# nianticlabs/simplerecon

Measured on AMD Instinct MI355X. Metric: depth frames/sec (640x480, 7 src views, 64 planes), higher is better.
Workload: dtype f32

## Files before the change

include/simplerecon_hip.h:

```cpp
#ifndef SIMPLERECON_HIP_H_
#define SIMPLERECON_HIP_H_

#include <stddef.h>
#include <stdint.h>

#ifdef __cplusplus
extern "C" {
#endif

#define SR_OK 0
#define SR_ERR_INVALID_ARGUMENT 1
#define SR_ERR_UNSUPPORTED 2
#define SR_ERR_WORKSPACE_TOO_SMALL 3
#define SR_ERR_HIP_BASE 1000

enum {
  SR_OPT_MLP_SPLIT = 0, SR_OPT_WINO_SPLIT, SR_OPT_WINO_XCD, SR_OPT_WINO_NT, SR_OPT_WINO_KSPLIT, SR_OPT_CONV_WINO,
  SR_OPT_CONV_TILE, SR_OPT_CONV_KSPLIT, SR_OPT_PW_NT, SR_OPT_PW_KS, SR_OPT_PT_CFG, SR_OPT_PT_KS, SR_OPT_DOT_LDS,
  SR_OPT_DOT_LDS_G, SR_OPT_DOT_LDS_CULL, SR_OPT_DOT_LDS_CAP, SR_OPT_UPSAMPLE_QUAD, SR_OPT_POOL_STREAM,
  SR_OPT_MLP_TILE,
  SR_OPT_COUNT
};
int sr_option_count(void);
const char* sr_option_name(int id);
int sr_option_id(const char* name);
int sr_option_get(int id, int* value);
int sr_option_set(int id, int value, int* previous );
int sr_option_default(int id, int* value);

int sr_abi_version(void);

const char* sr_target_arch(void);


size_t sr_volume_workspace_bytes(int B, int K, int C, int h, int w);

int sr_volume_prepare(const float* src, const float* K_src, const float* T_src_cur,
                      const float* T_cur_src, int B, int K, int C, int h, int w, void* workspace,
                      size_t workspace_bytes, void* stream);

int sr_dot_volume_sweep(const float* cur, const float* invK_cur, const float* planes, int64_t ps_b,
                        int64_t ps_d, int64_t ps_y, int64_t ps_x, int B, int K, int C, int h, int w,
                        int D, float* out_cv, int64_t cv_sb, int64_t cv_sd, int64_t cv_sp,
                        float* out_lowest, uint8_t* out_mask, void* workspace,
                        size_t workspace_bytes, void* stream);

int sr_conv3x3_wino_io_nhwc_fwd(const void* in, int64_t in_batch_stride, int in_pix_stride, const float* packed_u,
                                const float* bias, const void* residual, int64_t res_batch_stride, int res_pix_stride,
                                void* out, int64_t out_batch_stride, int out_pix_stride, int B, int H, int W, int Cin,
                                int Cout, float leaky_slope, int io_dtype, void* stream);
int sr_pw_conv_io_nhwc_fwd(const void* in, int64_t in_batch_stride, int in_pix_stride, const float* packed_w,
                           const float* bias, const void* residual, int64_t res_batch_stride, int res_pix_stride, void* out,
                           int64_t out_batch_stride, int out_pix_stride, int B, int HW, int Cin, int Cout, float act_code,
                           int io_dtype, void* stream);

size_t sr_pw_conv_tiled_workspace_bytes(int M, int Cin, int Cout);
int sr_pw_conv_tiled_plan(int M, int Cin, int Cout, int can_split, int* cfg, int* ks);
int sr_pw_conv_tiled_nhwc_fwd(const float* in, int in_pix_stride, const float* packed_w, const float* bias,
                              const float* gate, const float* residual, int res_pix_stride, float* out,
                              int out_pix_stride, int M, int HW, int Cin, int Cout, float act_code, void* workspace,
                              size_t workspace_bytes, void* stream);
int sr_pw_conv_supported(int Cin, int Cout);
int sr_pw_conv_plan(int B, int HW, int Cin, int Cout, int* nt, int* ks);
int sr_pw_conv_nhwc_fwd(const float* in, int64_t in_batch_stride, int in_pix_stride, const float* packed_w,
                        const float* bias, const float* gate, const float* residual, int64_t res_batch_stride,
                        int res_pix_stride, float* out, int64_t out_batch_stride, int out_pix_stride, int B, int HW,
                        int Cin, int Cout, float act_code, void* stream);

int sr_backproject_fwd(const float* depth, const float* invK, float* out_points, int B, int h, int w, void* stream);
int sr_project3d_fwd(const float* points, const float* K, const float* T, float* out, int B, int N, float eps,
                     void* stream);
int sr_backproject_bwd(const float* grad_points, const float* invK, float* grad_depth, int B, int h, int w, void* stream);
int sr_project3d_bwd(const float* grad_out, const float* points, const float* K, const float* T, float* grad_points, int B,
                     int N, float eps, void* stream);
int sr_pose_distance_fwd(const float* T, float* out, int n, void* stream);
int sr_camera_rays_fwd(const float* points, const float* T, float* out, int B, int N, int in_camera_frame, void* stream);

int sr_selftest_rcp(const float* x, float* out_fast, float* out_div, int n, void* stream);

int sr_dot_volume_fwd(const float* cur, const float* src, const float* K_src,
                      const float* T_src_cur, const float* invK_cur, const float* planes,
                      int64_t ps_b, int64_t ps_d, int64_t ps_y, int64_t ps_x, int B, int K, int C,
                      int h, int w, int D, float* out_cv, int64_t cv_sb, int64_t cv_sd,
                      int64_t cv_sp, float* out_lowest, uint8_t* out_mask, void* workspace,
                      size_t workspace_bytes, void* stream);

int sr_warp_features_fwd(const float* src, const float* K_src, const float* T_src_cur,
                         const float* invK_cur, const float* planes, int64_t ps_b, int64_t ps_d,
                         int64_t ps_y, int64_t ps_x, int B, int K, int C, int h, int w, int Dp,
                         float* out_world, float* out_depths, float* out_warped, float* out_mask,
                         float* out_pix, void* workspace, size_t workspace_bytes, void* stream);

size_t sr_mlp_volume_workspace_bytes(int B, int K, int C, int h, int w, int hidden);

int sr_mlp_pack_weights(const float* W1, const float* b1, const float* W2, const float* b2,
                        const float* W3, const float* b3, int hidden, int B, int K, int C, int h, int w,
                        void* workspace, size_t workspace_bytes, void* stream);

int sr_mlp_volume_sweep(const float* cur, const float* invK_cur, const float* planes, int64_t ps_b,
                        int64_t ps_d, int64_t ps_y, int64_t ps_x, float leaky_slope, int B, int K,
                        int C, int h, int w, int D, float* out_cv, int64_t cv_sb, int64_t cv_sd,
                        int64_t cv_sp, float* out_lowest, uint8_t* out_mask, void* workspace,
                        size_t workspace_bytes, void* stream);

int sr_mlp_volume_tile_shape(int h, int w, int* th, int* tw);

int sr_mlp_volume_fwd(const float* cur, const float* src, const float* K_src, const float* T_src_cur,
                      const float* T_cur_src, const float* invK_cur, const float* planes, int64_t ps_b,
                      int64_t ps_d, int64_t ps_y, int64_t ps_x, const float* W1, const float* b1,
                      const float* W2, const float* b2, const float* W3, const float* b3, int hidden,
                      float leaky_slope, int B, int K, int C, int h, int w, int D, float* out_cv,
                      int64_t cv_sb, int64_t cv_sd, int64_t cv_sp, float* out_lowest, uint8_t* out_mask,
                      int reserve_cus, void* workspace, size_t workspace_bytes, void* stream);


size_t sr_conv_packed_weight_floats(int Cout, int Cin, int ksize);

int sr_conv_pack_weights(const float* weight, int Cout, int Cin, int ksize, float* packed, void* stream);

int sr_conv2d_nhwc_fwd(const float* in, int64_t in_batch_stride, int in_pix_stride,
                       const float* packed_weight, const float* bias, const float* residual,
                       int64_t res_batch_stride, int res_pix_stride, float* out,
                       int64_t out_batch_stride, int out_pix_stride, int B, int H, int W, int Cin,
                       int Cout, int ksize, int stride, float leaky_slope, void* stream);

int sr_conv2d_replicate_nhwc_fwd(const float* in, int64_t in_batch_stride, int in_pix_stride,
                                 const float* packed_weight, const float* bias, const float* residual,
                                 int64_t res_batch_stride, int res_pix_stride, float* out,
                                 int64_t out_batch_stride, int out_pix_stride, int B, int H, int W, int Cin,
                                 int Cout, int ksize, int stride, float leaky_slope, void* stream);

#define SR_ACT_NONE (-1.0f)
#define SR_ACT_SILU (-2.0f)
int sr_conv2d_padded_nhwc_fwd(const float* in, int64_t in_batch_stride, int in_pix_stride,
                              const float* packed_weight, const float* bias, const float* residual,
                              int64_t res_batch_stride, int res_pix_stride, float* out,
                              int64_t out_batch_stride, int out_pix_stride, int B, int H, int W, int Cin,
                              int Cout, int ksize, int stride, int pad_top, int pad_left, int pad_bottom,
                              int pad_right, float leaky_slope, void* stream);

size_t sr_conv_splitk_workspace_bytes(int B, int H, int W, int Cin, int Cout, int ksize, int stride);
int sr_conv2d_splitk_nhwc_fwd(const float* in, int64_t in_batch_stride, int in_pix_stride,
                              const float* packed_weight, const float* bias, const float* residual,
                              int64_t res_batch_stride, int res_pix_stride, float* out,
                              int64_t out_batch_stride, int out_pix_stride, int B, int H, int W, int Cin,
                              int Cout, int ksize, int stride, float leaky_slope, void* workspace,
                              size_t workspace_bytes, void* stream);

size_t sr_wino_packed_weight_floats(int Cout, int Cin);
int sr_wino_pack_weights(const float* weight, int Cout, int Cin, float* packed, void* stream);
int sr_conv_prefers_wino(int B, int H, int W, int Cin, int Cout, int ksize, int stride);
int sr_conv3x3_wino_nhwc_fwd(const float* in, int64_t in_batch_stride, int in_pix_stride,
                             const float* packed_u, const float* bias, const float* residual,
                             int64_t res_batch_stride, int res_pix_stride, float* out,
                             int64_t out_batch_stride, int out_pix_stride, int B, int H, int W, int Cin,
                             int Cout, float leaky_slope, void* stream);

size_t sr_wino4_packed_weight_floats(int Cout, int Cin);
// ... 392 lines not shown
```

simplerecon_amd/_lib.py:

```python
import contextlib
import ctypes as C
import os

import torch

_HERE = os.path.dirname(os.path.abspath(__file__))
LIB_PATH = os.environ.get("SR_HIP_LIBRARY") or os.path.join(_HERE, "libsimplerecon_hip.so")
ABI_VERSION = 3

_lib = None

_p = C.c_void_p
_i = C.c_int
_i64 = C.c_int64
_f = C.c_float
_sz = C.c_size_t

SIGNATURES = {
    "sr_abi_version": (_i, []),
    "sr_option_count": (_i, []),
    "sr_option_name": (C.c_char_p, [_i]),
    "sr_option_id": (_i, [C.c_char_p]),
    "sr_option_get": (_i, [_i, C.POINTER(C.c_int)]),
    "sr_option_set": (_i, [_i, _i, C.POINTER(C.c_int)]),
    "sr_option_default": (_i, [_i, C.POINTER(C.c_int)]),
    "sr_target_arch": (C.c_char_p, []),
    "sr_volume_workspace_bytes": (_sz, [_i, _i, _i, _i, _i]),
    "sr_volume_prepare": (_i, [_p, _p, _p, _p, _i, _i, _i, _i, _i, _p, _sz, _p]),
    "sr_dot_volume_sweep": (_i, [_p, _p, _p, _i64, _i64, _i64, _i64, _i, _i, _i, _i, _i, _i,
                                 _p, _i64, _i64, _i64, _p, _p, _p, _sz, _p]),
    "sr_dot_volume_fwd": (_i, [_p, _p, _p, _p, _p, _p, _i64, _i64, _i64, _i64, _i, _i, _i, _i, _i, _i,
                               _p, _i64, _i64, _i64, _p, _p, _p, _sz, _p]),
    "sr_rgb_stem3x3s2_fwd": (_i, [_p, _i64, _i64, _i64, _i64, _p, _p, _p, _i64, _i, _i, _i, _i, _i, _i, _i, _i, _i, _f, _p]),
    "sr_se_gate2_fwd": (_i, [_p, _i, _i, _p, _p, _p, _p, _p, _p, _i, _i, _i, _p]),
    "sr_conv3x3_wino_io_nhwc_fwd": (_i, [_p, _i64, _i, _p, _p, _p, _i64, _i, _p, _i64, _i, _i, _i, _i, _i, _i, _f, _i, _p]),
    "sr_pw_conv_io_nhwc_fwd": (_i, [_p, _i64, _i, _p, _p, _p, _i64, _i, _p, _i64, _i, _i, _i, _i, _i, _f, _i, _p]),
    "sr_conv16_packed_weight_bytes": (_sz, [_i, _i, _i]),
    "sr_conv16_pack_weights": (_i, [_p, _i, _i, _i, _i, _p, _p]),
    "sr_conv16_supported": (_i, [_i, _i, _i, _i, _i, _i, _i]),
    "sr_conv16_prefers": (_i, [_i, _i, _i, _i, _i, _i, _i]),
    "sr_conv16_nhwc_fwd": (_i, [_p, _i64, _i, _p, _p, _p, _i64, _i, _p, _i64, _i, _i, _i, _i, _i, _i, _i, _i, _f, _i, _i, _p]),
    "sr_conv16_wgrad_supported": (_i, [_i, _i, _i, _i, _i, _i, _i]),
    "sr_conv16_wgrad_prefers": (_i, [_i, _i, _i, _i, _i, _i, _i]),
    "sr_conv16_wgrad_workspace_bytes": (_sz, [_i, _i, _i, _i, _i, _i, _i]),
    "sr_conv16_wgrad_nhwc": (_i, [_p, _i64, _i, _p, _i64, _i, _p, _i, _i, _i, _i, _i, _i, _i, _i, _p, _sz, _p]),
    "sr_act_bwd_bias16_workspace_bytes": (_sz, [_i64, _i]),
    "sr_act_bwd_bias16_nhwc": (_i, [_p, _i, _p, _p, _p, _i64, _i, _f, _i, _p, _sz, _p]),
    "sr_pw_conv_tiled_workspace_bytes": (_sz, [_i, _i, _i]),
    "sr_pw_conv_tiled_plan": (_i, [_i, _i, _i, _i, _p, _p]),
    "sr_pw_conv_tiled_nhwc_fwd": (_i, [_p, _i, _p, _p, _p, _p, _i, _p, _i, _i, _i, _i, _i, _f, _p, _sz, _p]),
    "sr_pw_conv_supported": (_i, [_i, _i]),
    "sr_pw_conv_plan": (_i, [_i, _i, _i, _i, _p, _p]),
    "sr_pw_conv_nhwc_fwd": (_i, [_p, _i64, _i, _p, _p, _p, _p, _i64, _i, _p, _i64, _i, _i, _i, _i, _i, _f, _p]),
    "sr_backproject_fwd": (_i, [_p, _p, _p, _i, _i, _i, _p]),
    "sr_project3d_fwd": (_i, [_p, _p, _p, _p, _i, _i, _f, _p]),
    "sr_backproject_bwd": (_i, [_p, _p, _p, _i, _i, _i, _p]),
    "sr_project3d_bwd": (_i, [_p, _p, _p, _p, _p, _i, _i, _f, _p]),
    "sr_pose_distance_fwd": (_i, [_p, _p, _i, _p]),
    "sr_camera_rays_fwd": (_i, [_p, _p, _p, _i, _i, _i, _p]),
    "sr_selftest_rcp": (_i, [_p, _p, _p, _i, _p]),
    "sr_warp_features_fwd": (_i, [_p, _p, _p, _p, _p, _i64, _i64, _i64, _i64, _i, _i, _i, _i, _i, _i,
                                  _p, _p, _p, _p, _p, _p, _sz, _p]),
    "sr_mlp_volume_workspace_bytes": (_sz, [_i, _i, _i, _i, _i, _i]),
    "sr_mlp_pack_weights": (_i, [_p, _p, _p, _p, _p, _p, _i, _i, _i, _i, _i, _i, _p, _sz, _p]),
    "sr_mlp_volume_sweep": (_i, [_p, _p, _p, _i64, _i64, _i64, _i64, _f, _i, _i, _i, _i, _i, _i,
                                 _p, _i64, _i64, _i64, _p, _p, _p, _sz, _p]),
    "sr_mlp_volume_tile_shape": (_i, [_i, _i, C.POINTER(C.c_int), C.POINTER(C.c_int)]),
    "sr_mlp_volume_fwd": (_i, [_p, _p, _p, _p, _p, _p, _p, _i64, _i64, _i64, _i64, _p, _p, _p, _p, _p, _p, _i,
                               _f, _i, _i, _i, _i, _i, _i, _p, _i64, _i64, _i64, _p, _p, _i, _p, _sz, _p]),
    "sr_conv_packed_weight_floats": (_sz, [_i, _i, _i]),
    "sr_conv_pack_weights": (_i, [_p, _i, _i, _i, _p, _p]),
    "sr_conv2d_nhwc_fwd": (_i, [_p, _i64, _i, _p, _p, _p, _i64, _i, _p, _i64, _i, _i, _i, _i, _i, _i, _i, _i, _f, _p]),
    "sr_conv2d_replicate_nhwc_fwd": (_i, [_p, _i64, _i, _p, _p, _p, _i64, _i, _p, _i64, _i, _i, _i, _i, _i, _i, _i, _i,
                                          _f, _p]),
    "sr_conv2d_padded_nhwc_fwd": (_i, [_p, _i64, _i, _p, _p, _p, _i64, _i, _p, _i64, _i, _i, _i, _i, _i, _i, _i, _i,
                                       _i, _i, _i, _i, _f, _p]),
    "sr_dwconv3x3_pool_bands": (_i, [_i]),
    "sr_dwconv3x3_nhwc_fwd": (_i, [_p, _i64, _i, _p, _p, _p, _i64, _i, _p, _i, _i, _i, _i, _i, _i, _i, _i, _i, _f,
                                   _p]),
    "sr_add_nhwc_fwd": (_i, [_p, _i64, _i, _p, _i64, _i, _p, _i64, _i, _i, _i, _i, _i, _p]),
    "sr_se_scale_nhwc_fwd": (_i, [_p, _i, _p, _p, _p, _p, _p, _p, _i64, _i, _p, _i64, _i, _p, _i, _i, _i, _i, _i,
                                  _p]),
    "sr_se_gate_fwd": (_i, [_p, _i, _i, _p, _p, _p, _p, _p, _i, _i, _i, _p]),
    "sr_scale_channels_nhwc_fwd": (_i, [_p, _i64, _i, _p, _p, _i64, _i, _i, _i, _i, _i, _p]),
    "sr_dot_volume_bwd_scratch_bytes": (_sz, [_i, _i, _i, _i, _i]),
    "sr_dot_volume_bwd": (_i, [_p, _i64, _i64, _i64, _p, _p, _p, _i64, _i64, _i64, _i64, _i, _i, _i, _i, _i, _i, _p, _p,
                               _p, _sz, _p, _sz, _p]),
    "sr_mlp_volume_bwd_scratch_bytes": (_sz, [_i, _i, _i, _i, _i, _i]),
    "sr_mlp_volume_bwd": (_i, [_p, _i64, _i64, _i64, _p, _p, _p, _i64, _i64, _i64, _i64, _p, _p, _p, _p, _p, _f, _i, _i,
                               _i, _i, _i, _i, _i, _p, _p, _p, _p, _p, _p, _p, _p, _p, _sz, _p, _sz, _p]),
    "sr_conv_wgrad_workspace_bytes": (_sz, [_i, _i, _i, _i, _i, _i, _i]),
    "sr_conv_wgrad_nhwc": (_i, [_p, _i64, _i, _p, _i64, _i, _p, _i, _i, _i, _i, _i, _i, _i, _p, _sz, _p]),
    "sr_bias_grad_nhwc": (_i, [_p, _i64, _i, _p, _i, _i, _i, _i, _p]),
    "sr_act_bwd": (_i, [_p, _p, _p, _i64, _f, _p]),
    "sr_act_bwd_bias_workspace_bytes": (_sz, [_i64, _i]),
    "sr_act_bwd_bias_nhwc": (_i, [_p, _p, _p, _p, _i64, _i, _f, _p, _sz, _p]),
    "sr_zero_stuff2x_nhwc": (_i, [_p, _i64, _i, _p, _i, _i, _i, _i, _i, _i, _p]),
    "sr_upsample2x_bwd_nhwc": (_i, [_p, _i64, _i, _p, _i64, _i, _i, _i, _i, _i, _p]),
    "sr_conv_flip_transpose_weights": (_i, [_p, _i, _i, _i, _p, _p]),
    "sr_mul_fwd": (_i, [_p, _p, _p, _i64, _p]),
    "sr_norm_workspace_bytes": (_sz, [_i, _i, _i, _i]),
    "sr_norm_stats_nhwc": (_i, [_p, _i64, _i, _i, _i, _i, _i, _p, _p, _p, _sz, _p]),
    "sr_norm_act_fwd_nhwc": (_i, [_p, _i64, _i, _p, _p, _f, _p, _p, _f, _i, _p, _i64, _i, _i, _i, _i, _p]),
    "sr_norm_act_bwd_nhwc": (_i, [_p, _i64, _i, _p, _i64, _i, _p, _p, _f, _p, _p, _f, _i, _i, _p, _i64, _i, _p, _p,
                                  _i, _i, _i, _p, _sz, _p]),
    "sr_rowsum_nhwc": (_i, [_p, _i64, _i, _p, _i64, _i, _i, _i, _i, _f, _p, _p, _sz, _p]),
    "sr_maxblurpool_bwd_workspace_bytes": (_sz, [_i, _i, _i, _i]),
    "sr_maxblurpool_bwd_nhwc": (_i, [_p, _i64, _i, _p, _i64, _i, _p, _i64, _i, _i, _i, _i, _i, _p, _sz, _p]),
    "sr_replicate_pad_nhwc_fwd": (_i, [_p, _i64, _i, _p, _i, _i, _i, _i, _i, _p]),
    "sr_replicate_pad_nhwc_bwd": (_i, [_p, _p, _i, _i, _i, _i, _i, _p]),
    "sr_im2col7x7s2_nhwc": (_i, [_p, _i64, _i64, _i64, _i64, _p, _i, _i, _i, _i, _p]),
    "sr_dwconv3x3_bwd_workspace_bytes": (_sz, [_i, _i, _i, _i]),
    "sr_dwconv3x3_bwd_nhwc": (_i, [_p, _i64, _i, _p, _i64, _i, _p, _p, _p, _i, _i, _i, _i, _i, _i, _i, _i, _i, _p, _sz,
                                   _p]),
    "sr_scale_bwd_nhwc": (_i, [_p, _i64, _i, _p, _p, _f, _p, _i, _i, _i, _p]),
    "sr_small_linear_fwd": (_i, [_p, _p, _p, _p, _p, _i, _i, _i, _f, _p]),
    "sr_small_linear_bwd": (_i, [_p, _p, _p, _p, _p, _p, _p, _i, _i, _i, _f, _p]),
    "sr_act_in_bwd": (_i, [_p, _p, _p, _i64, _f, _p]),
    "sr_add_act_fwd": (_i, [_p, _p, _p, _p, _i64, _f, _p]),
    "sr_conv_wgrad_padded_workspace_bytes": (_sz, [_i, _i, _i, _i, _i, _i]),
# ... 288 lines not shown
```

simplerecon_amd/csrc/sr_mlp_volume.hip:

```cpp
#include <stdlib.h>
#include <string.h>

#include "sr_buffer.h"
#include "sr_view.h"

#define SR_HID 128
#define SR_VIEW_SLOTS 24
#define SR_INV_FIXED 20
#define SR_PLANE_CHUNK 8

static inline int sr_mlp_steps_var(int K) { return (SR_VIEW_SLOTS / 2) * K; }
static inline int sr_mlp_steps_inv(int K) { return (SR_INV_FIXED + 3 * K + 1) / 2; }
static inline int sr_mlp_steps1(int K) { return sr_mlp_steps_var(K) + sr_mlp_steps_inv(K); }
#define SR_MLP_STEPS2 65

static inline size_t sr_mlp_packed_floats(int K) { return (size_t)(sr_mlp_steps1(K) + SR_MLP_STEPS2) * 256 + 128 + 4; }

__global__ void sr_mlp_pack_kernel(const float* __restrict__ W1, const float* __restrict__ b1,
                                   const float* __restrict__ W2, const float* __restrict__ b2,
                                   const float* __restrict__ W3, const float* __restrict__ b3,
                                   float* __restrict__ packed, int K, int C) {
  const int steps_var = (SR_VIEW_SLOTS / 2) * K;
  const int steps1 = steps_var + (SR_INV_FIXED + 3 * K + 1) / 2;
  const int Cin = C * (K + 1) + 10 * K + 4;
  const int o_cur = K * C, o_mask = o_cur + C, o_z = o_mask + K, o_d = o_z + K, o_dot = o_d + 1;
  const int o_ang = o_dot + K, o_cray = o_ang + K, o_sray = o_cray + 3, o_pd = o_sray + 3 * K;
  const int o_rm = o_pd + K, o_tm = o_rm + K;
  const int total = (steps1 + SR_MLP_STEPS2) * 256 + 128 + 1;
  for (int e = blockIdx.x * blockDim.x + threadIdx.x; e < total; e += gridDim.x * blockDim.x) {
    float v = 0.0f;
    if (e < steps1 * 256) {
      const int t = e >> 8, lane = (e >> 2) & 63, mt = e & 3;
      const int row = 32 * mt + (lane & 31);
      int col = -1;
      if (t < steps_var) {
        const int slot = 2 * t + (lane >> 5);
        const int k = slot / SR_VIEW_SLOTS, s = slot - k * SR_VIEW_SLOTS;
        if (s < 16) col = k * C + s;
        else if (s == 16) col = o_mask + k;
        else if (s == 17) col = o_z + k;
        else if (s == 18) col = o_dot + k;
        else if (s == 19) col = o_ang + k;
        else if (s < 23) col = o_sray + 3 * k + (s - 20);
        else col = (k == 0) ? o_d : -1;
      } else {
        const int u = 2 * (t - steps_var) + (lane >> 5);
        if (u < 16) col = o_cur + u;
        else if (u < 19) col = o_cray + (u - 16);
        else if (u == 19) col = -2;
        else if (u < SR_INV_FIXED + 3 * K) {
          const int k = (u - SR_INV_FIXED) / 3, i = (u - SR_INV_FIXED) - 3 * k;
          col = (i == 0 ? o_pd : (i == 1 ? o_rm : o_tm)) + k;
        }
      }
      v = (col >= 0) ? W1[(size_t)row * Cin + col] : (col == -2 ? b1[row] : 0.0f);
    } else if (e < (steps1 + SR_MLP_STEPS2) * 256) {
      const int e2 = e - steps1 * 256;
      const int t = e2 >> 8, lane = (e2 >> 2) & 63, mt = e2 & 3;
      const int row = 32 * mt + (lane & 31);
      if (t < 64) {
        const int m = t >> 4, r = t & 15;
        const int f = 32 * m + (r & 3) + 8 * (r >> 2) + 4 * (lane >> 5);
        v = W2[(size_t)row * SR_HID + f];
      } else {
        v = (lane < 32) ? b2[row] : 0.0f;
      }
    } else if (e < (steps1 + SR_MLP_STEPS2) * 256 + 128) {
      const int i = e - (steps1 + SR_MLP_STEPS2) * 256;
      const int half = i >> 6, mt = (i >> 4) & 3, r = i & 15;
      v = W3[32 * mt + (r & 3) + 8 * (r >> 2) + 4 * half];
    } else {
      v = b3[0];
    }
    packed[e] = v;
  }
}


struct SrMlpParams {
  const float* cur;
  const float* src_nhwc;
  const float* invK;
  const float* geom;
  const float* packed;
  SrPlanes planes;
  SrVolumeOut out;
  int B, K, h, w, D;
  int tiles;
  int tiles_x;
  int th_log2, tw_log2;
  int chunk, chunks;
  int vec_store;
  float inv_w, inv_h, slope;
};

__device__ __forceinline__ bool sr_mlp_lane_pixel(const SrMlpParams& p, int tile, int lane, int& y, int& x) {
  if (p.tiles_x) {
    const int ty = tile / p.tiles_x, tx = tile - ty * p.tiles_x;
    const int ly = (ty << p.th_log2) + (lane >> p.tw_log2);
    const int lx = (tx << p.tw_log2) + (lane & ((1 << p.tw_log2) - 1));
    y = min(ly, p.h - 1);
    x = min(lx, p.w - 1);
    return ly < p.h && lx < p.w;
  }
  const int N = p.h * p.w, pix = tile * 64 + lane;
  const int pc = min(pix, N - 1);
  y = pc / p.w;
  x = pc - y * p.w;
  return pix < N;
}

__device__ __forceinline__ void sr_swap_halves(float fa, float fb, float& bP, float& bQ) {
  auto r = __builtin_amdgcn_permlane32_swap(__float_as_uint(fa), __float_as_uint(fb), false, false);
  bP = __uint_as_float(r[0]);
  bQ = __uint_as_float(r[1]);
}

#define SR_MFMA(a, b, c) __builtin_amdgcn_mfma_f32_32x32x2f32((a), (b), (c), 0, 0, 0)

__device__ __forceinline__ void sr_l1_step(f32x16 (&acc)[2][4], const float4 wA, float fa, float fb) {
  float bP, bQ;
  sr_swap_halves(fa, fb, bP, bQ);
  acc[0][0] = SR_MFMA(wA.x, bP, acc[0][0]);
  acc[1][0] = SR_MFMA(wA.x, bQ, acc[1][0]);
  acc[0][1] = SR_MFMA(wA.y, bP, acc[0][1]);
  acc[1][1] = SR_MFMA(wA.y, bQ, acc[1][1]);
  acc[0][2] = SR_MFMA(wA.z, bP, acc[0][2]);
  acc[1][2] = SR_MFMA(wA.z, bQ, acc[1][2]);
  acc[0][3] = SR_MFMA(wA.w, bP, acc[0][3]);
  acc[1][3] = SR_MFMA(wA.w, bQ, acc[1][3]);
}

__device__ __forceinline__ void sr_l1_step_init(f32x16 (&acc)[2][4], const f32x16 (&hc)[2][4], const float4 wA,
                                                float fa, float fb) {
  float bP, bQ;
  sr_swap_halves(fa, fb, bP, bQ);
  acc[0][0] = SR_MFMA(wA.x, bP, hc[0][0]);
  acc[1][0] = SR_MFMA(wA.x, bQ, hc[1][0]);
  acc[0][1] = SR_MFMA(wA.y, bP, hc[0][1]);
  acc[1][1] = SR_MFMA(wA.y, bQ, hc[1][1]);
  acc[0][2] = SR_MFMA(wA.z, bP, hc[0][2]);
  acc[1][2] = SR_MFMA(wA.z, bQ, hc[1][2]);
  acc[0][3] = SR_MFMA(wA.w, bP, hc[0][3]);
  acc[1][3] = SR_MFMA(wA.w, bQ, hc[1][3]);
}

__device__ __forceinline__ int sr_opaque(bool flag) {
  int v = __builtin_amdgcn_readfirstlane((int)flag);
  asm volatile("" : "+s"(v));
  return v;
}

#define SR_LDS_W3_FLOATS 256

template <bool W1_LDS, bool W2_LDS>
__global__ __launch_bounds__(256, 1) void sr_mlp_volume_kernel(SrMlpParams p) {
  extern __shared__ __attribute__((aligned(16))) float lds[];
  constexpr int C = 16;
  constexpr int VS = SR_VIEW_SLOTS / 2;
  const int lane = threadIdx.x & 63;
  const int steps_var = VS * p.K;
  const int steps1 = steps_var + (SR_INV_FIXED + 3 * p.K + 1) / 2;
  const float4* gW1 = reinterpret_cast<const float4*>(p.packed);
  const float4* gW1inv = gW1 + (size_t)steps_var * 64;
  const float4* gW2 = gW1 + (size_t)steps1 * 64;
  const float* gW3 = p.packed + (size_t)(steps1 + SR_MLP_STEPS2) * 256;

  for (int i = threadIdx.x; i < 129; i += blockDim.x) lds[i] = gW3[i];
  constexpr int W2_FLOATS = W2_LDS ? SR_MLP_STEPS2 * 256 : 0;
  if (W2_LDS) {
    float4* l4 = reinterpret_cast<float4*>(lds + SR_LDS_W3_FLOATS);
    for (int i = threadIdx.x; i < SR_MLP_STEPS2 * 64; i += blockDim.x) l4[i] = gW2[i];
  }
  if (W1_LDS) {
    float4* l4 = reinterpret_cast<float4*>(lds + SR_LDS_W3_FLOATS + W2_FLOATS);
    for (int i = threadIdx.x; i < steps_var * 64; i += blockDim.x) l4[i] = gW1[i];
  }
  __syncthreads();
  const float4* W1p = W1_LDS ? reinterpret_cast<const float4*>(lds + SR_LDS_W3_FLOATS + W2_FLOATS) : gW1;

  const int N = p.h * p.w;
  const long nunits = (long)p.B * p.tiles * p.chunks;
  constexpr int WPB = 4;
  const int wid = __builtin_amdgcn_readfirstlane(threadIdx.x >> 6);
  long wave0 = (long)blockIdx.x * WPB + wid;
  long nwaves = (long)gridDim.x * WPB;
  long unit_end = nunits;
  if ((gridDim.x & 7) == 0) {
    const long u8 = (nunits + 7) / 8;
    const int xcd = blockIdx.x & 7;
    nwaves = (long)(gridDim.x >> 3) * WPB;
    wave0 = xcd * u8 + (long)(blockIdx.x >> 3) * WPB + wid;
    unit_end = min(nunits, (xcd + 1) * u8);
  }
  const int half = lane >> 5;

  const int rot = (int)max(1L, nwaves / p.chunks);
  for (long unit = wave0; unit < unit_end; unit += nwaves) {
    const long tb = unit / p.chunks;
    const int chunk = (int)((unit % p.chunks + tb / rot) % p.chunks);
    const int tile = (int)(tb % p.tiles);
    const int b = (int)(tb / p.tiles);
    const int j0 = chunk * p.chunk, j1 = min(p.D, j0 + p.chunk);
    int y, x;
    const bool in_image = sr_mlp_lane_pixel(p, tile, lane, y, x);
    const int pc = y * p.w + x;
    const int pix = in_image ? pc : -1;
    const bool active = pix >= 0;
    const float* plane_ptr = p.planes.ptr + b * p.planes.sb + y * p.planes.sy + x * p.planes.sx;
    const float* geom_b = p.geom + (size_t)b * p.K * SR_GEOM_STRIDE;
    const float* src_b = p.src_nhwc + (size_t)b * p.K * N * C;

    float cur[C];
#pragma unroll
    for (int c = 0; c < C; ++c) cur[c] = p.cur[((size_t)b * C + c) * N + pc];

    float r0, r1, r2;
    {
#pragma clang fp contract(off)
      const float* iK = p.invK + 16 * (size_t)b;
      const float px = (float)x + 0.5f, py = (float)y + 0.5f;
      r0 = iK[0] * px + iK[1] * py + iK[2];
      r1 = iK[4] * px + iK[5] * py + iK[6];
      r2 = iK[8] * px + iK[9] * py + iK[10];
    }
    float cr0, cr1, cr2, crn0, crn1, crn2;
    {
#pragma clang fp contract(off)
      const float d0 = plane_ptr[0];
      const float X0 = d0 * r0, X1 = d0 * r1, X2 = d0 * r2;
      const float cden = fmaxf(sqrtf((X0 * X0 + X1 * X1) + X2 * X2), 1e-12f);
      cr0 = X0 / cden; cr1 = X1 / cden; cr2 = X2 / cden;
      const float n1 = fmaxf(sqrtf((cr0 * cr0 + cr1 * cr1) + cr2 * cr2), 1e-5f);
      crn0 = cr0 / n1; crn1 = cr1 / n1; crn2 = cr2 / n1;
    }

    f32x16 hc[2][4];
#pragma unroll
    for (int g = 0; g < 2; ++g)
#pragma unroll
      for (int m = 0; m < 4; ++m)
#pragma unroll
        for (int r = 0; r < 16; ++r) hc[g][m][r] = 0.0f;
    {
      const float4* wi = gW1inv + lane;
#pragma unroll
      for (int t = 0; t < 8; ++t) sr_l1_step(hc, wi[t * 64], cur[2 * t], cur[2 * t + 1]);
      sr_l1_step(hc, wi[8 * 64], cr0, cr1);
      sr_l1_step(hc, wi[9 * 64], cr2, 1.0f);
      const int npose = 3 * p.K;
#pragma unroll 1
      for (int u = 0; u < npose; u += 2) {
        const int ka = u / 3, ia = u - 3 * ka, kb = (u + 1) / 3, ib = (u + 1) - 3 * kb;
        const float fa = geom_b[ka * SR_GEOM_STRIDE + 15 + ia];
        const float fb = (u + 1 < npose) ? geom_b[kb * SR_GEOM_STRIDE + 15 + ib] : 0.0f;
// ... 615 lines not shown
      }
      if (active) {
        if (!p.vec_store) p.out.cv[b * p.out.sb + j * p.out.sd + (int64_t)pix * p.out.sp] = cost;
        if (j == p.D - 1 && p.out.mask) p.out.mask[(size_t)b * N + pix] = (uint8_t)(any_depth && any_bounds);
      }
    }
    if (p.vec_store && active) {
      float* row = p.out.cv + b * p.out.sb + (int64_t)pix * p.out.sp + j0;
#pragma unroll
      for (int q = 0; q < SR_PLANE_CHUNK; q += 4) {
        if (j0 + q + 4 <= j1) *reinterpret_cast<float4*>(row + q) = make_float4(cst[q], cst[q + 1], cst[q + 2], cst[q + 3]);
        else {
#pragma unroll
          for (int i = 0; i < 4; ++i)
            if (j0 + q + i < j1) row[q + i] = cst[q + i];
        }
      }
    }
  }
}

static int sr_mlp_split_mode() { return sr_opt(SR_OPT_MLP_SPLIT); }

__global__ void sr_argmax_planes_kernel(const float* __restrict__ cv, int64_t sb, int64_t sd, int64_t sp,
                                        SrPlanes planes, int h, int w, int D, float* __restrict__ lowest) {
  const int N = h * w;
  const int pix = blockIdx.x * blockDim.x + threadIdx.x;
  const int b = blockIdx.y;
  if (pix >= N) return;
  const int y = pix / w, x = pix - y * w;
  const float* c = cv + b * sb + (int64_t)pix * sp;
  float best = c[0];
  int bj = 0;
  int j = 1;
  for (; j + 8 <= D; j += 8) {
    float v[8];
#pragma unroll
    for (int u = 0; u < 8; ++u) v[u] = c[(int64_t)(j + u) * sd];
#pragma unroll
    for (int u = 0; u < 8; ++u)
      if (v[u] > best || (v[u] != v[u] && best == best)) { best = v[u]; bj = j + u; }
  }
  for (; j < D; ++j) {
    const float v = c[(int64_t)j * sd];
    if (v > best || (v != v && best == best)) { best = v; bj = j; }
  }
  lowest[(size_t)b * N + pix] = planes.ptr[b * planes.sb + bj * planes.sd + y * planes.sy + x * planes.sx];
}


extern "C" size_t sr_mlp_volume_workspace_bytes(int B, int K, int C, int h, int w, int hidden) {
  (void)hidden;
  if (B < 0 || K < 0) return 0;
  return sr_volume_workspace_bytes(B, K, C, h, w) + sr_align_up(sr_mlp_packed_floats(K) * sizeof(float), 256) + 256;
}

extern "C" int sr_mlp_volume_tile_shape(int h, int w, int* th, int* tw) {
  if (h <= 0 || w <= 0 || !th || !tw) return SR_ERR_INVALID_ARGUMENT;
  const int mode = sr_opt(SR_OPT_MLP_TILE);
  if (mode < 0 || mode > 4) return SR_ERR_INVALID_ARGUMENT;
  *th = 1; *tw = 64;
  if (mode >= 2) { *th = 1 << (mode - 1); *tw = 64 >> (mode - 1); }
  if (mode == 0) {
    const int64_t flat = ((int64_t)h * w + 63) / 64;
    for (int t = 8; t >= 2; t >>= 1) {
      const int64_t tiles = (int64_t)((h + t - 1) / t) * ((w + 64 / t - 1) / (64 / t));
      if (100 * tiles <= 101 * flat) { *th = t; *tw = 64 / t; break; }
    }
  }
  return SR_OK;
}

static float* sr_ws_packed(void* workspace, int B, int K, int C, int h, int w) {
  return (float*)sr_align_up((size_t)workspace + sr_volume_workspace_bytes(B, K, C, h, w), 256);
}

static int sr_mlp_volume_sweep_reserved(const float* cur, const float* invK_cur, const float* planes, int64_t ps_b,
                                        int64_t ps_d, int64_t ps_y, int64_t ps_x, float leaky_slope, int B, int K,
                                        int C, int h, int w, int D, float* out_cv, int64_t cv_sb, int64_t cv_sd,
                                        int64_t cv_sp, float* out_lowest, uint8_t* out_mask, int reserve_cus,
                                        void* workspace, size_t workspace_bytes, void* stream_) {
  if (B < 0 || K <= 0 || C <= 0 || h <= 0 || w <= 0 || D <= 0) return SR_ERR_INVALID_ARGUMENT;
  if (B == 0) return SR_OK;
  if (!cur || !invK_cur || !planes || !out_cv || !workspace) return SR_ERR_INVALID_ARGUMENT;
  if (C != 16) return SR_ERR_UNSUPPORTED;
  if (!(leaky_slope > 0.0f && leaky_slope < 1.0f)) return SR_ERR_UNSUPPORTED;
  if (workspace_bytes < sr_mlp_volume_workspace_bytes(B, K, C, h, w, SR_HID)) return SR_ERR_WORKSPACE_TOO_SMALL;
  hipStream_t stream = (hipStream_t)stream_;
  const int N = h * w;

  SrMlpParams p;
  p.cur = cur; p.src_nhwc = sr_ws_src_nhwc(workspace, B, K); p.invK = invK_cur; p.geom = sr_ws_geom(workspace);
  p.packed = sr_ws_packed(workspace, B, K, C, h, w);
  p.planes = {planes, ps_b, ps_d, ps_y, ps_x};
  p.out = {out_cv, cv_sb, cv_sd, cv_sp, out_lowest, out_mask};
  p.B = B; p.K = K; p.h = h; p.w = w; p.D = D;
  int th, tw;
  if (sr_mlp_volume_tile_shape(h, w, &th, &tw)) return SR_ERR_INVALID_ARGUMENT;
  p.th_log2 = __builtin_ctz(th); p.tw_log2 = __builtin_ctz(tw);
  p.tiles_x = th == 1 ? 0 : (w + tw - 1) / tw;
  p.tiles = th == 1 ? (N + 63) / 64 : p.tiles_x * ((h + th - 1) / th);
  p.inv_w = (float)(1.0 / (double)w);
  p.inv_h = (float)(1.0 / (double)h);
  p.slope = leaky_slope;

  int cus = sr_device_cus();
  if (reserve_cus > 0 && cus - reserve_cus >= 8) cus -= reserve_cus;
  const long waves = 4L * cus;
  double best_cost = 1e30;
  int best = 1;
  for (int c = SR_PLANE_CHUNK; c >= 1; c >>= 1) {
    const long units = (long)B * p.tiles * ((D + c - 1) / c);
    const long rounds = (units + waves - 1) / waves;
    const double cost = (double)rounds * (c * 1192.0 + 168.0);
    if (cost < best_cost) { best_cost = cost; best = c; }
  }
  p.chunk = best;
  p.chunks = (D + best - 1) / best;
  p.vec_store = (cv_sd == 1) && (p.chunk % 4 == 0) && sr_rows_aligned(out_cv, cv_sb, cv_sp, 15, 4);
  const long nunits = (long)B * p.tiles * p.chunks;
  const int blocks = (int)((nunits + 3) / 4 < cus ? (nunits + 3) / 4 : cus);
  const size_t w3_bytes = SR_LDS_W3_FLOATS * sizeof(float);
  const size_t w1_bytes = (size_t)sr_mlp_steps_var(K) * 1024;
  const size_t w2_bytes = (size_t)SR_MLP_STEPS2 * 1024;
  const size_t lds_max = 160 * 1024;
  const int split = sr_mlp_split_mode();
  if (split < 0) return SR_ERR_INVALID_ARGUMENT;
  if (split) {
    const size_t bytes = ((size_t)SR_SPL_TAB + SR_SPL_W2_WORDS + (size_t)K * SR_SPL_VIEW_WORDS) * 4;
    if (bytes > lds_max) return SR_ERR_UNSUPPORTED;
    const void* fn = split == 1 ? (const void*)sr_mlp_volume_split_kernel<1> : (const void*)sr_mlp_volume_split_kernel<2>;
    if (hipError_t e = sr_allow_lds(fn, bytes)) return sr_hip_rc(e);
    if (split == 1) hipLaunchKernelGGL((sr_mlp_volume_split_kernel<1>), dim3(blocks), dim3(256), bytes, stream, p);
    else hipLaunchKernelGGL((sr_mlp_volume_split_kernel<2>), dim3(blocks), dim3(256), bytes, stream, p);
    int rc = sr_hip_rc(hipGetLastError());
    if (rc) return rc;
    if (out_lowest) rc = sr_launch_argmax_planes(out_cv, cv_sb, cv_sd, cv_sp, p.planes, B, h, w, D, out_lowest, stream);
    return rc;
  }
#define SR_MLP_LAUNCH(L1, L2, BYTES)                                                                              \
  {                                                                                                               \
           \
    if (hipError_t e = sr_allow_lds((const void*)sr_mlp_volume_kernel<L1, L2>, (BYTES))) return sr_hip_rc(e);     \
    hipLaunchKernelGGL((sr_mlp_volume_kernel<L1, L2>), dim3(blocks), dim3(256), (BYTES), stream, p);              \
  }
  if (w1_bytes + w2_bytes + w3_bytes <= lds_max) SR_MLP_LAUNCH(true, true, w1_bytes + w2_bytes + w3_bytes)
  else if (w1_bytes + w3_bytes <= lds_max) SR_MLP_LAUNCH(true, false, w1_bytes + w3_bytes)
  else SR_MLP_LAUNCH(false, true, w2_bytes + w3_bytes + 4 * SR_PLANE_CHUNK * 64 * sizeof(float))
#undef SR_MLP_LAUNCH
  int rc = sr_hip_rc(hipGetLastError());
  if (rc) return rc;
  if (out_lowest) rc = sr_launch_argmax_planes(out_cv, cv_sb, cv_sd, cv_sp, p.planes, B, h, w, D, out_lowest, stream);
  return rc;
}

extern "C" int sr_mlp_volume_sweep(const float* cur, const float* invK_cur, const float* planes, int64_t ps_b,
                                   int64_t ps_d, int64_t ps_y, int64_t ps_x, float leaky_slope, int B, int K,
                                   int C, int h, int w, int D, float* out_cv, int64_t cv_sb, int64_t cv_sd,
                                   int64_t cv_sp, float* out_lowest, uint8_t* out_mask, void* workspace,
                                   size_t workspace_bytes, void* stream_) {
  return sr_mlp_volume_sweep_reserved(cur, invK_cur, planes, ps_b, ps_d, ps_y, ps_x, leaky_slope, B, K, C, h, w, D, out_cv,
                                      cv_sb, cv_sd, cv_sp, out_lowest, out_mask, 0, workspace, workspace_bytes, stream_);
}

int sr_launch_argmax_planes(const float* cv, int64_t sb, int64_t sd, int64_t sp, SrPlanes planes, int B, int h, int w,
                            int D, float* lowest, hipStream_t stream) {
  hipLaunchKernelGGL(sr_argmax_planes_kernel, dim3((h * w + 63) / 64, B), dim3(64), 0, stream, cv, sb, sd, sp,
                     planes, h, w, D, lowest);
  return sr_hip_rc(hipGetLastError());
}

extern "C" int sr_mlp_pack_weights(const float* W1, const float* b1, const float* W2, const float* b2,
                                   const float* W3, const float* b3, int hidden, int B, int K, int C, int h, int w,
                                   void* workspace, size_t workspace_bytes, void* stream_) {
  if (!W1 || !b1 || !W2 || !b2 || !W3 || !b3 || !workspace || K <= 0) return SR_ERR_INVALID_ARGUMENT;
  if (hidden != SR_HID || C != 16) return SR_ERR_UNSUPPORTED;
  if (workspace_bytes < sr_mlp_volume_workspace_bytes(B, K, C, h, w, hidden)) return SR_ERR_WORKSPACE_TOO_SMALL;
  const int split = sr_mlp_split_mode();
  if (split < 0) return SR_ERR_INVALID_ARGUMENT;
  float* packed = sr_ws_packed(workspace, B, K, C, h, w);
  if (split == 1) hipLaunchKernelGGL((sr_mlp_pack_split_kernel<1>), dim3(64), dim3(256), 0, (hipStream_t)stream_, W1, b1, W2, b2, W3, b3, packed, K, C);
  else if (split == 2) hipLaunchKernelGGL((sr_mlp_pack_split_kernel<2>), dim3(64), dim3(256), 0, (hipStream_t)stream_, W1, b1, W2, b2, W3, b3, packed, K, C);
  else hipLaunchKernelGGL(sr_mlp_pack_kernel, dim3(64), dim3(256), 0, (hipStream_t)stream_, W1, b1, W2, b2, W3, b3, packed, K, C);
  return sr_hip_rc(hipGetLastError());
}

extern "C" int sr_mlp_volume_fwd(const float* cur, const float* src, const float* K_src, const float* T_src_cur,
                                 const float* T_cur_src, const float* invK_cur, const float* planes, int64_t ps_b,
                                 int64_t ps_d, int64_t ps_y, int64_t ps_x, const float* W1, const float* b1,
                                 const float* W2, const float* b2, const float* W3, const float* b3, int hidden,
                                 float leaky_slope, int B, int K, int C, int h, int w, int D, float* out_cv,
                                 int64_t cv_sb, int64_t cv_sd, int64_t cv_sp, float* out_lowest, uint8_t* out_mask,
                                 int reserve_cus, void* workspace, size_t workspace_bytes, void* stream_) {
  if (B < 0 || K <= 0 || C <= 0 || h <= 0 || w <= 0 || D <= 0 || reserve_cus < 0) return SR_ERR_INVALID_ARGUMENT;
  if (B == 0) return SR_OK;
  if (!T_cur_src) return SR_ERR_INVALID_ARGUMENT;
  if (hidden != SR_HID || C != 16) return SR_ERR_UNSUPPORTED;
  if (workspace_bytes < sr_mlp_volume_workspace_bytes(B, K, C, h, w, hidden)) return SR_ERR_WORKSPACE_TOO_SMALL;
// ... 9 lines not shown
```

simplerecon_amd/csrc/sr_options.hip:

```cpp
#include <atomic>
#include <map>
#include <mutex>
#include <utility>
#include <stdlib.h>
#include <string.h>

#include "sr_common.h"

namespace {

struct OptDef { const char* name; int dflt; int kind; };
const OptDef kDefs[SR_OPT_COUNT] = {
    {"SR_MLP_SPLIT", 0, 1},       {"SR_WINO_SPLIT", 0, 1},     {"SR_WINO_XCD", 1, 0},        {"SR_WINO_NT", 0, 0},
    {"SR_WINO_KSPLIT", 0, 0},     {"SR_CONV_WINO", 1, 0},      {"SR_CONV_TILE", 0, 0},       {"SR_CONV_KSPLIT", 1, 0},
    {"SR_PW_NT", 0, 0},           {"SR_PW_KS", 0, 0},          {"SR_PT_CFG", -1, 0},         {"SR_PT_KS", 0, 0},
    {"SR_DOT_LDS", 1, 0},         {"SR_DOT_LDS_G", 0, 0},      {"SR_DOT_LDS_CULL", 1, 0},    {"SR_DOT_LDS_CAP", 634, 0},
    {"SR_UPSAMPLE_QUAD", 1, 0},   {"SR_POOL_STREAM", 1, 0},    {"SR_MLP_TILE", 0, 2},
};
std::atomic<int> g_val[SR_OPT_COUNT];
std::once_flag g_once;

int parse(const OptDef& d, const char* e) {
  if (d.kind == 1) {
    if (!e || !*e || !strcmp(e, "0") || !strcmp(e, "off") || !strcmp(e, "fp32")) return 0;
    if (!strcmp(e, "bf16")) return 1;
    if (!strcmp(e, "f16") || !strcmp(e, "fp16")) return 2;
    return -1;
  }
  if (d.kind == 2) {
    static const char* const names[] = {"auto", "flat", "2x32", "4x16", "8x8"};
    if (!e || !*e) return d.dflt;
    for (int i = 0; i < 5; ++i)
      if (!strcmp(e, names[i])) return i;
    return -1;
  }
  return (e && *e) ? atoi(e) : d.dflt;
}

void init() {
  for (int i = 0; i < SR_OPT_COUNT; ++i) {
    const char* e = getenv(kDefs[i].name);
    g_val[i].store(e ? parse(kDefs[i], e) : kDefs[i].dflt, std::memory_order_relaxed);
  }
}

}

int sr_opt(int id) {
  std::call_once(g_once, init);
  return g_val[id].load(std::memory_order_relaxed);
}

extern "C" int sr_option_count(void) { return SR_OPT_COUNT; }

extern "C" const char* sr_option_name(int id) { return (id >= 0 && id < SR_OPT_COUNT) ? kDefs[id].name : nullptr; }

extern "C" int sr_option_id(const char* name) {
  if (!name) return -1;
  for (int i = 0; i < SR_OPT_COUNT; ++i)
    if (!strcmp(kDefs[i].name, name)) return i;
  return -1;
}

extern "C" int sr_option_get(int id, int* value) {
  if (id < 0 || id >= SR_OPT_COUNT || !value) return SR_ERR_INVALID_ARGUMENT;
  *value = sr_opt(id);
  return SR_OK;
}

extern "C" int sr_option_set(int id, int value, int* previous) {
// ... 39 lines not shown
```

Measured before the change: 324.5.

## Use per-XCD atomic ticket queues for dynamic MLP volume work distribution

Replaces the static round-robin assignment of (tile, plane-chunk) units to waves in the MLP cost-volume kernel with a dynamic work queue. Each XCD gets its own atomic ticket counter in the workspace, reset by a memset before launch. The chunk-size planner gains a per-unit prologue cost term for the queue mode and is factored into a shared plan function, with a host helper exposing the unit order. This targets load imbalance and tail effects, at the cost of one atomic per unit, an extra memset launch, and possibly smaller chunks.

```diff
diff --git a/include/simplerecon_hip.h b/include/simplerecon_hip.h
--- a/include/simplerecon_hip.h
+++ b/include/simplerecon_hip.h
@@ -18,7 +18,7 @@
   SR_OPT_MLP_SPLIT = 0, SR_OPT_WINO_SPLIT, SR_OPT_WINO_XCD, SR_OPT_WINO_NT, SR_OPT_WINO_KSPLIT, SR_OPT_CONV_WINO,
   SR_OPT_CONV_TILE, SR_OPT_CONV_KSPLIT, SR_OPT_PW_NT, SR_OPT_PW_KS, SR_OPT_PT_CFG, SR_OPT_PT_KS, SR_OPT_DOT_LDS,
   SR_OPT_DOT_LDS_G, SR_OPT_DOT_LDS_CULL, SR_OPT_DOT_LDS_CAP, SR_OPT_UPSAMPLE_QUAD, SR_OPT_POOL_STREAM,
-  SR_OPT_MLP_TILE,
+  SR_OPT_MLP_TILE, SR_OPT_MLP_QUEUE,
   SR_OPT_COUNT
 };
 int sr_option_count(void);
@@ -104,6 +104,8 @@
                         size_t workspace_bytes, void* stream);
 
 int sr_mlp_volume_tile_shape(int h, int w, int* th, int* tw);
+
+int sr_mlp_volume_unit_order(int B, int h, int w, int D, int reserve_cus, int* plan, int* units, size_t capacity);
 
 int sr_mlp_volume_fwd(const float* cur, const float* src, const float* K_src, const float* T_src_cur,
                       const float* T_cur_src, const float* invK_cur, const float* planes, int64_t ps_b,
diff --git a/simplerecon_amd/_lib.py b/simplerecon_amd/_lib.py
--- a/simplerecon_amd/_lib.py
+++ b/simplerecon_amd/_lib.py
@@ -66,6 +66,7 @@
     "sr_mlp_volume_sweep": (_i, [_p, _p, _p, _i64, _i64, _i64, _i64, _f, _i, _i, _i, _i, _i, _i,
                                  _p, _i64, _i64, _i64, _p, _p, _p, _sz, _p]),
     "sr_mlp_volume_tile_shape": (_i, [_i, _i, C.POINTER(C.c_int), C.POINTER(C.c_int)]),
+    "sr_mlp_volume_unit_order": (_i, [_i, _i, _i, _i, _i, C.POINTER(C.c_int), C.POINTER(C.c_int), _sz]),
     "sr_mlp_volume_fwd": (_i, [_p, _p, _p, _p, _p, _p, _p, _i64, _i64, _i64, _i64, _p, _p, _p, _p, _p, _p, _i,
                                _f, _i, _i, _i, _i, _i, _i, _p, _i64, _i64, _i64, _p, _p, _i, _p, _sz, _p]),
     "sr_conv_packed_weight_floats": (_sz, [_i, _i, _i]),
diff --git a/simplerecon_amd/csrc/sr_mlp_units.h b/simplerecon_amd/csrc/sr_mlp_units.h
--- /dev/null
+++ b/simplerecon_amd/csrc/sr_mlp_units.h
@@ -0,0 +1,42 @@
+#pragma once
+#include <stdint.h>
+
+#if defined(__HIPCC__) || defined(__CUDACC__)
+#define SR_UNITS_FN __host__ __device__ static inline
+#else
+#define SR_UNITS_FN static inline
+#endif
+
+SR_UNITS_FN int sr_mlp_queues(int blocks) { return (blocks & 7) == 0 ? 8 : 1; }
+
+SR_UNITS_FN void sr_mlp_queue_range(int pairs, int nq, int q, int* first, int* count) {
+  const int lo = (int)((int64_t)pairs * q / nq), hi = (int)((int64_t)pairs * (q + 1) / nq);
+  *first = lo;
+  *count = hi - lo;
+}
+
+SR_UNITS_FN int sr_mlp_ticket_unit(int first, int count, int chunks, uint32_t t, int* pair, int* chunk) {
+  if (count <= 0 || t >= (uint32_t)count * (uint32_t)chunks) return 0;
+  const uint32_t row = t / (uint32_t)count;
+  *pair = first + (int)(t - row * (uint32_t)count);
+  *chunk = chunks - 1 - (int)row;
+  return 1;
+}
+
+SR_UNITS_FN int sr_mlp_queue_fits(int64_t pairs, int chunks, int64_t waves) {
+  return pairs > 0 && chunks > 0 && pairs * chunks + waves < ((int64_t)1 << 31);
+}
+
+SR_UNITS_FN void sr_mlp_static_range(int64_t nunits, int nq, int q, int64_t* first, int64_t* end) {
+  if (nq == 1) { *first = 0; *end = nunits; return; }
+  const int64_t u8 = (nunits + nq - 1) / nq;
+  *first = q * u8;
+  *end = nunits < (q + 1) * u8 ? nunits : (q + 1) * u8;
+}
+
+SR_UNITS_FN void sr_mlp_static_unit(int64_t unit, int chunks, int64_t nwaves, int* pair, int* chunk) {
+  const int64_t rot = nwaves / chunks > 1 ? nwaves / chunks : 1;
+  const int64_t tb = unit / chunks;
+  *chunk = (int)((unit % chunks + tb / rot) % chunks);
+  *pair = (int)tb;
+}
diff --git a/simplerecon_amd/csrc/sr_mlp_volume.hip b/simplerecon_amd/csrc/sr_mlp_volume.hip
--- a/simplerecon_amd/csrc/sr_mlp_volume.hip
+++ b/simplerecon_amd/csrc/sr_mlp_volume.hip
@@ -2,6 +2,7 @@
 #include <string.h>
 
 #include "sr_buffer.h"
+#include "sr_mlp_units.h"
 #include "sr_view.h"
 
 #define SR_HID 128
@@ -92,6 +93,8 @@
   int chunk, chunks;
   int vec_store;
   float inv_w, inv_h, slope;
+  int queue;
+  unsigned* tickets;
 };
 
 __device__ __forceinline__ bool sr_mlp_lane_pixel(const SrMlpParams& p, int tile, int lane, int& y, int& x) {
@@ -183,24 +186,31 @@
   const long nunits = (long)p.B * p.tiles * p.chunks;
   constexpr int WPB = 4;
   const int wid = __builtin_amdgcn_readfirstlane(threadIdx.x >> 6);
-  long wave0 = (long)blockIdx.x * WPB + wid;
-  long nwaves = (long)gridDim.x * WPB;
-  long unit_end = nunits;
-  if ((gridDim.x & 7) == 0) {
-    const long u8 = (nunits + 7) / 8;
-    const int xcd = blockIdx.x & 7;
-    nwaves = (long)(gridDim.x >> 3) * WPB;
-    wave0 = xcd * u8 + (long)(blockIdx.x >> 3) * WPB + wid;
-    unit_end = min(nunits, (xcd + 1) * u8);
-  }
+  const int nq = sr_mlp_queues(gridDim.x);
+  const int xcd = nq == 8 ? blockIdx.x & 7 : 0;
+  const long nwaves = (long)(gridDim.x / nq) * WPB;
+  long unit, unit_end;
+  sr_mlp_static_range(nunits, nq, xcd, &unit, &unit_end);
+  unit += (long)(blockIdx.x / nq) * WPB + wid;
+  int q_first, q_pairs;
+  sr_mlp_queue_range(p.B * p.tiles, nq, xcd, &q_first, &q_pairs);
+  unsigned* const ticket_ctr = p.tickets + xcd;
   const int half = lane >> 5;
 
-  const int rot = (int)max(1L, nwaves / p.chunks);
-  for (long unit = wave0; unit < unit_end; unit += nwaves) {
-    const long tb = unit / p.chunks;
-    const int chunk = (int)((unit % p.chunks + tb / rot) % p.chunks);
-    const int tile = (int)(tb % p.tiles);
-    const int b = (int)(tb / p.tiles);
+  for (;;) {
+    int pair, chunk;
+    if (p.queue) {
+      unsigned t = 0;
+      if (lane == 0) t = atomicAdd(ticket_ctr, 1u);
+      t = __builtin_amdgcn_readfirstlane(t);
+      if (!sr_mlp_ticket_unit(q_first, q_pairs, p.chunks, t, &pair, &chunk)) break;
+    } else {
+      if (unit >= unit_end) break;
+      sr_mlp_static_unit(unit, p.chunks, nwaves, &pair, &chunk);
+      unit += nwaves;
+    }
+    const int b = pair / p.tiles;
+    const int tile = pair - b * p.tiles;
     const int j0 = chunk * p.chunk, j1 = min(p.D, j0 + p.chunk);
     int y, x;
     const bool in_image = sr_mlp_lane_pixel(p, tile, lane, y, x);
@@ -922,7 +932,7 @@
 extern "C" size_t sr_mlp_volume_workspace_bytes(int B, int K, int C, int h, int w, int hidden) {
   (void)hidden;
   if (B < 0 || K < 0) return 0;
-  return sr_volume_workspace_bytes(B, K, C, h, w) + sr_align_up(sr_mlp_packed_floats(K) * sizeof(float), 256) + 256;
+  return sr_volume_workspace_bytes(B, K, C, h, w) + sr_align_up(sr_mlp_packed_floats(K) * sizeof(float), 256) + 256 + 256;
 }
 
 extern "C" int sr_mlp_volume_tile_shape(int h, int w, int* th, int* tw) {
@@ -943,6 +953,73 @@
 
 static float* sr_ws_packed(void* workspace, int B, int K, int C, int h, int w) {
   return (float*)sr_align_up((size_t)workspace + sr_volume_workspace_bytes(B, K, C, h, w), 256);
+}
+
+static unsigned* sr_ws_tickets(void* workspace, int B, int K, int C, int h, int w) {
+  return (unsigned*)((char*)sr_ws_packed(workspace, B, K, C, h, w) + sr_align_up(sr_mlp_packed_floats(K) * sizeof(float), 256));
+}
+
+struct SrMlpPlan { int th, tw, tiles_x, tiles, chunk, chunks, blocks, queue; };
+
+static int sr_mlp_plan(int B, int h, int w, int D, int reserve_cus, bool may_queue, SrMlpPlan* pl) {
+  if (sr_mlp_volume_tile_shape(h, w, &pl->th, &pl->tw)) return SR_ERR_INVALID_ARGUMENT;
+  const int N = h * w;
+  pl->tiles_x = pl->th == 1 ? 0 : (w + pl->tw - 1) / pl->tw;
+  pl->tiles = pl->th == 1 ? (N + 63) / 64 : pl->tiles_x * ((h + pl->th - 1) / pl->th);
+  int cus = sr_device_cus();
+  if (reserve_cus > 0 && cus - reserve_cus >= 8) cus -= reserve_cus;
+  const long waves = 4L * cus;
+  const int mode = sr_opt(SR_OPT_MLP_QUEUE);
+  if (mode < 0 || mode > SR_PLANE_CHUNK || (mode & (mode - 1))) return SR_ERR_INVALID_ARGUMENT;
+  pl->queue = may_queue && mode != 0 && sr_mlp_queue_fits((int64_t)B * pl->tiles, D, waves);
+  const double SR_UNIT_PROLOGUE = 432.0;
+  double best_cost = 1e30;
+  int best = 1;
+  for (int c = SR_PLANE_CHUNK; c >= (pl->queue ? 4 : 1); c >>= 1) {
+    const long units = (long)B * pl->tiles * ((D + c - 1) / c);
+    const double unit_cost = c * 1192.0 + 168.0;
+    const double cost = pl->queue ? ((double)units / waves + 1.0) * (unit_cost + SR_UNIT_PROLOGUE)
+                                  : (double)((units + waves - 1) / waves) * unit_cost;
+    if (cost < best_cost) { best_cost = cost; best = c; }
+  }
+  if (pl->queue && mode > 1) best = mode;
+  pl->chunk = best;
+  pl->chunks = (D + best - 1) / best;
+  const long nunits = (long)B * pl->tiles * pl->chunks;
+  pl->blocks = (int)((nunits + 3) / 4 < cus ? (nunits + 3) / 4 : cus);
+  return SR_OK;
+}
+
+extern "C" int sr_mlp_volume_unit_order(int B, int h, int w, int D, int reserve_cus, int* plan, int* units, size_t capacity) {
+  if (B <= 0 || h <= 0 || w <= 0 || D <= 0 || reserve_cus < 0 || !plan) return SR_ERR_INVALID_ARGUMENT;
+  SrMlpPlan pl;
+  if (int rc = sr_mlp_plan(B, h, w, D, reserve_cus, sr_mlp_split_mode() == 0, &pl)) return rc;
+  const int nq = sr_mlp_queues(pl.blocks), pairs = B * pl.tiles;
+  const long nwaves = (long)(pl.blocks / nq) * 4, nunits = (long)pairs * pl.chunks;
+  plan[0] = pl.queue; plan[1] = nq; plan[2] = (int)nwaves; plan[3] = pl.chunk; plan[4] = pl.chunks; plan[5] = pl.tiles;
+  plan[6] = (int)nunits; plan[7] = pl.blocks;
+  if (!units) return SR_OK;
+  if (capacity < (size_t)nunits) return SR_ERR_INVALID_ARGUMENT;
+  int* row = units;
+  for (int q = 0; q < nq; ++q) {
+    if (pl.queue) {
+      int first, count, pair, chunk;
+      sr_mlp_queue_range(pairs, nq, q, &first, &count);
+      for (uint32_t t = 0; sr_mlp_ticket_unit(first, count, pl.chunks, t, &pair, &chunk); ++t, row += 5) {
+        row[0] = q; row[1] = (int)t; row[2] = pair / pl.tiles; row[3] = pair % pl.tiles; row[4] = chunk;
+      }
+    } else {
+      int64_t first, end;
+      sr_mlp_static_range(nunits, nq, q, &first, &end);
+      for (long wv = 0; wv < nwaves; ++wv)
+        for (int64_t u = first + wv; u < end; u += nwaves, row += 5) {
+          int pair, chunk;
+          sr_mlp_static_unit(u, pl.chunks, nwaves, &pair, &chunk);
+          row[0] = q; row[1] = (int)wv; row[2] = pair / pl.tiles; row[3] = pair % pl.tiles; row[4] = chunk;
+        }
+    }
+  }
+  return (row - units) == 5 * nunits ? SR_OK : SR_ERR_INVALID_ARGUMENT;
 }
 
 static int sr_mlp_volume_sweep_reserved(const float* cur, const float* invK_cur, const float* planes, int64_t ps_b,
@@ -957,7 +1034,6 @@
   if (!(leaky_slope > 0.0f && leaky_slope < 1.0f)) return SR_ERR_UNSUPPORTED;
   if (workspace_bytes < sr_mlp_volume_workspace_bytes(B, K, C, h, w, SR_HID)) return SR_ERR_WORKSPACE_TOO_SMALL;
   hipStream_t stream = (hipStream_t)stream_;
-  const int N = h * w;
 
   SrMlpParams p;
   p.cur = cur; p.src_nhwc = sr_ws_src_nhwc(workspace, B, K); p.invK = invK_cur; p.geom = sr_ws_geom(workspace);
@@ -965,37 +1041,26 @@
   p.planes = {planes, ps_b, ps_d, ps_y, ps_x};
   p.out = {out_cv, cv_sb, cv_sd, cv_sp, out_lowest, out_mask};
   p.B = B; p.K = K; p.h = h; p.w = w; p.D = D;
-  int th, tw;
-  if (sr_mlp_volume_tile_shape(h, w, &th, &tw)) return SR_ERR_INVALID_ARGUMENT;
-  p.th_log2 = __builtin_ctz(th); p.tw_log2 = __builtin_ctz(tw);
-  p.tiles_x = th == 1 ? 0 : (w + tw - 1) / tw;
-  p.tiles = th == 1 ? (N + 63) / 64 : p.tiles_x * ((h + th - 1) / th);
+  const int split = sr_mlp_split_mode();
+  if (split < 0) return SR_ERR_INVALID_ARGUMENT;
+  SrMlpPlan pl;
+  if (int rc = sr_mlp_plan(B, h, w, D, reserve_cus, !split, &pl)) return rc;
+  p.th_log2 = __builtin_ctz(pl.th); p.tw_log2 = __builtin_ctz(pl.tw);
+  p.tiles_x = pl.tiles_x;
+  p.tiles = pl.tiles;
   p.inv_w = (float)(1.0 / (double)w);
   p.inv_h = (float)(1.0 / (double)h);
   p.slope = leaky_slope;
-
-  int cus = sr_device_cus();
-  if (reserve_cus > 0 && cus - reserve_cus >= 8) cus -= reserve_cus;
-  const long waves = 4L * cus;
-  double best_cost = 1e30;
-  int best = 1;
-  for (int c = SR_PLANE_CHUNK; c >= 1; c >>= 1) {
-    const long units = (long)B * p.tiles * ((D + c - 1) / c);
-    const long rounds = (units + waves - 1) / waves;
-    const double cost = (double)rounds * (c * 1192.0 + 168.0);
-    if (cost < best_cost) { best_cost = cost; best = c; }
-  }
-  p.chunk = best;
-  p.chunks = (D + best - 1) / best;
+  p.chunk = pl.chunk;
+  p.chunks = pl.chunks;
   p.vec_store = (cv_sd == 1) && (p.chunk % 4 == 0) && sr_rows_aligned(out_cv, cv_sb, cv_sp, 15, 4);
-  const long nunits = (long)B * p.tiles * p.chunks;
-  const int blocks = (int)((nunits + 3) / 4 < cus ? (nunits + 3) / 4 : cus);
+  p.queue = pl.queue;
+  p.tickets = sr_ws_tickets(workspace, B, K, C, h, w);
+  const int blocks = pl.blocks;
   const size_t w3_bytes = SR_LDS_W3_FLOATS * sizeof(float);
   const size_t w1_bytes = (size_t)sr_mlp_steps_var(K) * 1024;
   const size_t w2_bytes = (size_t)SR_MLP_STEPS2 * 1024;
   const size_t lds_max = 160 * 1024;
-  const int split = sr_mlp_split_mode();
-  if (split < 0) return SR_ERR_INVALID_ARGUMENT;
   if (split) {
     const size_t bytes = ((size_t)SR_SPL_TAB + SR_SPL_W2_WORDS + (size_t)K * SR_SPL_VIEW_WORDS) * 4;
     if (bytes > lds_max) return SR_ERR_UNSUPPORTED;
@@ -1014,6 +1079,8 @@
     if (hipError_t e = sr_allow_lds((const void*)sr_mlp_volume_kernel<L1, L2>, (BYTES))) return sr_hip_rc(e);     \
     hipLaunchKernelGGL((sr_mlp_volume_kernel<L1, L2>), dim3(blocks), dim3(256), (BYTES), stream, p);              \
   }
+  if (p.queue)
+    if (hipError_t e = hipMemsetAsync(p.tickets, 0, 8 * sizeof(unsigned), stream)) return sr_hip_rc(e);
   if (w1_bytes + w2_bytes + w3_bytes <= lds_max) SR_MLP_LAUNCH(true, true, w1_bytes + w2_bytes + w3_bytes)
   else if (w1_bytes + w3_bytes <= lds_max) SR_MLP_LAUNCH(true, false, w1_bytes + w3_bytes)
   else SR_MLP_LAUNCH(false, true, w2_bytes + w3_bytes + 4 * SR_PLANE_CHUNK * 64 * sizeof(float))
diff --git a/simplerecon_amd/csrc/sr_options.hip b/simplerecon_amd/csrc/sr_options.hip
--- a/simplerecon_amd/csrc/sr_options.hip
+++ b/simplerecon_amd/csrc/sr_options.hip
@@ -16,6 +16,7 @@
     {"SR_PW_NT", 0, 0},           {"SR_PW_KS", 0, 0},          {"SR_PT_CFG", -1, 0},         {"SR_PT_KS", 0, 0},
     {"SR_DOT_LDS", 1, 0},         {"SR_DOT_LDS_G", 0, 0},      {"SR_DOT_LDS_CULL", 1, 0},    {"SR_DOT_LDS_CAP", 634, 0},
     {"SR_UPSAMPLE_QUAD", 1, 0},   {"SR_POOL_STREAM", 1, 0},    {"SR_MLP_TILE", 0, 2},
+    {"SR_MLP_QUEUE", 1, 0},
 };
 std::atomic<int> g_val[SR_OPT_COUNT];
 std::once_flag g_once;
```

Result: no change. 324.6 (median of 2 runs) (+0.0%).
